# NILOIDE/A.I.gar

Hardware: NVIDIA B200
Metric: env_steps_per_sec (higher is better)
Workload: dtype f64

## Files before the change

a.i.gar_b200/csrc/agar_b200.cu:

```cuda
#include <cuda_runtime.h>
#include <math.h>
#include <stdio.h>
#include <stdlib.h>
#include <string.h>

#include "../../include/agar_b200.h"
#include "../../include/agar_layout.h"
#include "agar_bots.cuh"
#include "agar_dev.cuh"
#include "agar_simple.cuh"

extern __shared__ __align__(16) uint8_t g_smem[];

__device__ __forceinline__ void stage_in(const DevParams& P, const uint8_t* state, int env0, int n_here, bool zero) {
    const int chunks = (int)(P.L.record_bytes / 8);
    const int total = n_here * chunks;
    const uint2* src = (const uint2*)(state + (size_t)env0 * P.L.record_bytes);
    for (int i = threadIdx.x; i < total; i += blockDim.x) {
        int e = i / chunks, w = i - e * chunks;
        uint2 v = zero ? make_uint2(0u, 0u) : src[i];
        ((uint2*)(g_smem + (size_t)e * P.rec_stride))[w] = v;
    }
    __syncthreads();
}
// ... 94 lines not shown
#ifdef AGAR_PHASE_CLOCKS
            c.clk_t = clock64(), c.clk_env = env;
#endif
            if (psync) __syncthreads();
            CLK_MARK(0);
            const int f = n_frames > 0 ? it % n_frames : 0, d = n_frames > 0 ? it / n_frames : 0;
            const bool emit = last || (f == 0 && (flags & KF_OBS_BEFORE));
            if (active && !last && c.lane == 0) c.h->n_events = 0;
            if (FULL && K > 1 && active && !last) {
                update_all_fovs(c, P);
                c.fov_done = true;
                CLK_MARK(8);
                if (K * P.L.cell_cap > W) build_live_cells(c, P);
                CLK_MARK(11);
            }
            for (int k = 0; k < K; ++k) {
                if (psync_bots && k > 0) __syncthreads();
                if (active) {
                    if (!FULL || P.cfg.bot_type[k] == AGAR_BOT_NN) {
                        nn_turn_begin<W, FULL>(c, P, k, (emit && obs_env) ? obs_env + (size_t)k * SL : nullptr);
                        if (last) continue;
                        if (c.lane == 0) {
                            float act[4] = {0.f, 0.f, 0.f, 0.f};
                            if (c.pl[k].bot.need_action) {
                                if (flags & KF_RANDOM_ACTIONS) {
                                    uint32_t w[4];
                                    philox(dec_base + (uint32_t)d, 7u, c.env_id, (uint32_t)k, (uint32_t)P.seed,
                                           (uint32_t)(P.seed >> 32), w);
                                    for (int i = 0; i < 4; ++i) act[i] = (float)(w[i] >> 8) * (1.0f / 16777216.0f);
                                } else {
                                    const float* ap = actions + ((size_t)env * A + k) * 4;
                                    for (int i = 0; i < 4; ++i) act[i] = ap[i];
                                }
                            }
                            nn_turn_end(c, P, k, act);
                        }
                        c.t.sync();
                    } else if (FULL && !last) {
                        CLK_MARK(1);
                        scripted_turn(c, P, k);
                        CLK_MARK(7);
                    }
                }
            }
            if (last) break;
            CLK_MARK(1);
            c.fov_done = false, c.n_live = -1;
            for (int ph = 0; ph < AGAR_FIELD_PHASES; ++ph) {
                if (ph == 0 ? psync : psync_field) __syncthreads();
                if (ph == 0) CLK_MARK(2);
                if (active) field_update_phase<W, FULL>(c, P, ph);
                CLK_MARK(3 + ph);
            }
            if (active) {
                if (c.lane == 0) c.h->frame += 1;
                c.t.sync();
            }
            CLK_MARK(12);
        }
        if (active && c.lane == 0 && (P.turn_reward || P.turn_done))
            for (int a = 0; a < A; ++a) {
                if (P.turn_reward) P.turn_reward[(size_t)env * A + a] = (float)c.pl[a].bot.last_reward;
                if (P.turn_done) P.turn_done[(size_t)env * A + a] = (uint8_t)c.pl[a].bot.exp_done;
            }
    }
    if (P.stage == 1) stage_out(P, state, env0, n_here);
    if (P.stage >= 2) {
        __syncthreads();
        pel_cache_copy(P, state, env0, n_here, tiles, false);
    }
    export_tail(P, obs, env0, n_here);
}


struct SimplePlan {
    int frame_sync;
    int strideB;
    int grid_off;
    int obs_warps;
    int snap_off;
    int snap_stride;
};

enum { SB_PHYS = 1, SB_FULL = 2, SB_EMPTY = 4 };
struct SimpleSnap {
    double fov_x, fov_y, fov_size, mass;
    int32_t out;
    int32_t pad;
};
__host__ __device__ constexpr int simple_max_threads(int W) { return W == 8 ? 352 : 256; }
constexpr int SIMPLE_OBS_MIN_FRAMES = 4;
constexpr int SIMPLE_OBS_LANES = 4;
constexpr int SIMPLE_OBS_WARPS = 4;

template <int ID>
DEV void named_bar_sync(int n) { asm volatile("bar.sync %0, %1;" ::"n"(ID), "r"(n) : "memory"); }
template <int ID>
DEV void named_bar_arrive(int n) { asm volatile("bar.arrive %0, %1;" ::"n"(ID), "r"(n) : "memory"); }

template <int W, bool OBSW>
__global__ void __launch_bounds__(OBSW ? simple_max_threads(W) : 256, W == 1 ? 2 : 1)
k_simple(const __grid_constant__ DevParams P, const SimplePlan SP, uint8_t* __restrict__ state, const float* __restrict__ actions,
         float* __restrict__ obs, int n_frames, int n_dec, int flags, uint32_t dec_base) {
    const int phys_threads = blockDim.x - 32 * SP.obs_warps;
    const int per = phys_threads / W;
    const int env0 = blockIdx.x * per;
    const int n_here = min(per, P.n_envs - env0);
    const int rec_words = (int)(P.L.record_bytes / 4), pel_word = (int)(P.L.off_pellets / 4);
    const int tail_words = rec_words - pel_word;
    {
        for (int i = threadIdx.x; i < per * tail_words; i += blockDim.x) {
            int e = i / tail_words, w = i - e * tail_words;
            int es = e < n_here ? e : n_here - 1;
            const uint32_t* src = (const uint32_t*)(state + (size_t)(env0 + es) * P.L.record_bytes) + pel_word;
            *(uint32_t*)(g_smem + (size_t)e * SP.strideB + w * 4) = src[w];
        }
    }
    __syncthreads();
    auto snap = [&](int buf, int e) { return g_smem + SP.snap_off + (size_t)(buf * per + e) * SP.snap_stride; };
    if (OBSW && (int)threadIdx.x >= phys_threads) {
        constexpr int WO = SIMPLE_OBS_LANES;
        const int ot = ((int)threadIdx.x - phys_threads) / WO, osub = threadIdx.x % WO, n_ot = 32 * SP.obs_warps / WO;
        for (int d = 0; d < n_dec; ++d) {
            const int buf = d & 1;
            if (buf) named_bar_sync<SB_FULL + 1>(blockDim.x);
            else named_bar_sync<SB_FULL>(blockDim.x);
            for (int base = 0; base < per; base += n_ot) {
                const int e = min(base + ot, per - 1);
                const SimpleSnap* sn = (const SimpleSnap*)snap(buf, e);
                SReg r;
                r.fov_x = sn->fov_x, r.fov_y = sn->fov_y, r.fov_size = sn->fov_size, r.mass = sn->mass;
                SPtr q;
                q.pel = (uint32_t*)(sn + 1);
                q.grid = (uint32_t*)(g_smem + (size_t)e * SP.strideB + SP.grid_off);
                const bool out = base + ot < per && sn->out != 0;
                s_encode<WO>(r, q, P, out, out ? obs + (size_t)(env0 + e) * P.L.state_len : nullptr, osub);
            }
            if (d + 2 < n_dec) {
                if (buf) named_bar_arrive<SB_EMPTY + 1>(blockDim.x);
                else named_bar_arrive<SB_EMPTY>(blockDim.x);
            }
        }
        if (flags & KF_OBS_AFTER) __syncthreads();
    } else {
        const int slot = threadIdx.x / W, sub = threadIdx.x % W;
        const bool valid = slot < n_here;
        const int env = env0 + (valid ? slot : n_here - 1);
        const uint32_t env_id = (uint32_t)(P.first_env + (uint64_t)env);
        uint8_t* rec = state + (size_t)env * P.L.record_bytes;
        uint8_t* b = g_smem + (size_t)slot * SP.strideB;
        SPtr q;
        q.h = (AgarEnvHeader*)(rec + P.L.off_header);
        q.p = (AgarPlayer*)(rec + P.L.off_players);
        q.c = (AgarCell*)(rec + P.L.off_cells);
        q.pel = (uint32_t*)b;
        q.ev = (AgarEvent*)(b + (P.L.off_events - P.L.off_pellets));
        q.grid = SP.grid_off ? (uint32_t*)(b + SP.grid_off) : nullptr;
        SReg r;
        s_load(r, q);
        float* row = (obs != nullptr && valid) ? obs + (size_t)env * P.L.state_len : nullptr;
        auto frame_bar = [&]() {
            if (OBSW) named_bar_sync<SB_PHYS>(phys_threads);
            else __syncthreads();
        };
        for (int d = 0; d < n_dec; ++d) {
            if (OBSW && SP.obs_warps) {
                const int d_o = s_turn_begin(r, P);
                if (d_o) s_observe_state(r, P);
                const int buf = d & 1;
                if (d >= 2) {
                    if (buf) named_bar_sync<SB_EMPTY + 1>(blockDim.x);
                    else named_bar_sync<SB_EMPTY>(blockDim.x);
                }
                uint8_t* sn = snap(buf, slot);
                uint32_t* pool = (uint32_t*)(sn + sizeof(SimpleSnap));
                for (int i = sub; i < P.L.pellet_cap; i += W) pool[i] = q.pel[i];
                if (sub == 0) {
                    SimpleSnap* h = (SimpleSnap*)sn;
                    h->fov_x = r.fov_x, h->fov_y = r.fov_y, h->fov_size = r.fov_size, h->mass = r.mass;
                    h->out = d_o != 0 && row != nullptr;
                }
                if (buf) named_bar_arrive<SB_FULL + 1>(blockDim.x);
                else named_bar_arrive<SB_FULL>(blockDim.x);
            } else if (flags & KF_OBS_BEFORE) {
                int d_o = s_turn_begin(r, P);
                s_observe<W>(r, q, P, d_o != 0, row, sub);
            }
            for (int f = 0; f < n_frames; ++f) {
                if (SP.frame_sync == 1 || SP.frame_sync == 4) frame_bar();
                if (SP.frame_sync == 2) __syncwarp();
                r.n_events = 0;
                int d_o = s_turn_begin(r, P);
                s_observe<W>(r, q, P, d_o != 0, nullptr, sub);
                float act[4] = {0.f, 0.f, 0.f, 0.f};
                if (r.need_action) {
                    if (flags & KF_RANDOM_ACTIONS) {
                        uint32_t w[4];
                        philox(dec_base + (uint32_t)d, 7u, env_id, 0u, (uint32_t)P.seed, (uint32_t)(P.seed >> 32), w);
                        for (int i = 0; i < 4; ++i) act[i] = (float)(w[i] >> 8) * (1.0f / 16777216.0f);
                    } else {
                        const float* ap = actions + (size_t)env * 4;
                        for (int i = 0; i < 4; ++i) act[i] = ap[i];
                    }
                }
                double speed_pow;
                s_turn_end<W>(r, P, act, sub, speed_pow);
                if (SP.frame_sync == 4) frame_bar();
                s_field_update<W>(r, q, P, env_id, sub, speed_pow);
            }
        }
        if (flags & KF_OBS_AFTER) {
            if (OBSW) __syncthreads();
            int d_o = s_turn_begin(r, P);
            s_observe<W>(r, q, P, d_o != 0, row, sub);
        }
        if (valid && sub == 0) {
            s_store(r, q);
            if (P.turn_reward) P.turn_reward[env] = (float)r.last_reward;
            if (P.turn_done) P.turn_done[env] = (uint8_t)r.exp_done;
        }
    }
    __syncthreads();
    for (int i = threadIdx.x; i < n_here * tail_words; i += blockDim.x) {
        int e = i / tail_words, w = i - e * tail_words;
        uint32_t* dst = (uint32_t*)(state + (size_t)(env0 + e) * P.L.record_bytes) + pel_word;
        dst[w] = *(const uint32_t*)(g_smem + (size_t)e * SP.strideB + w * 4);
    }
    export_tail(P, obs, env0, n_here);
}

template <int W, bool FULL>
__global__ void __launch_bounds__(1024)
k_init(const __grid_constant__ DevParams P, uint8_t* __restrict__ state, const uint8_t* __restrict__ mask, int mode) {
    const int tiles = blockDim.x / W;
    const int env0 = blockIdx.x * tiles;
    const int n_here = min(tiles, P.n_envs - env0);
    if (P.stage == 1)
        stage_in(P, state, env0, n_here, mode == 0);
    else if (mode == 0) {
        const int chunks = (int)(P.L.record_bytes / 8);
        uint2* dst = (uint2*)(state + (size_t)env0 * P.L.record_bytes);
        for (int i = threadIdx.x; i < n_here * chunks; i += blockDim.x) dst[i] = make_uint2(0u, 0u);
        __syncthreads();
    }
    if (P.stage >= 2) pel_cache_copy(P, state, env0, n_here, tiles, true);
    const int tile_id = threadIdx.x / W;
    if (tile_id < n_here && (mask == nullptr || mode == 0 || mask[env0 + tile_id])) {
        Ctx<W> c(cg::tiled_partition<W>(cg::this_thread_block()));
        bind_ctx(c, P, tile_id, tiles, env0 + tile_id, state);
        const int K = P.L.n_players;
        if (mode == 0 || mode == 1) {
            if (mode == 1) {
                for (int i = c.lane; i < P.L.pellet_cap; i += W) c.pel[i] = 0;
                AgarFatPellet zf = {};
                for (int i = c.lane; i < P.L.fat_cap; i += W) c.fat[i] = zf;
                AgarMote zm = {};
                for (int i = c.lane; i < P.L.blob_cap; i += W) c.blob[i] = zm;
                for (int i = c.lane; i < P.L.virus_cap; i += W) c.vir[i] = zm;
                c.t.sync();
            }
            if (c.lane == 0) {
                if (mode == 0) {
                    for (int k = 0; k < K; ++k) {
                        AgarPlayer* p = &c.pl[k];
                        p->alive = 1;
                        p->cmd_x = p->cmd_y = -1;
                        p->bot.type = P.cfg.bot_type[k];
                    }
                } else {
                    c.h->n_events = 0;
                    c.h->n_pellets = c.h->n_fat = c.h->n_blobs = c.h->n_viruses = 0;
                    c.h->n_dead = 0;
                    for (int i = 0; i < AGAR_MAX_PLAYERS; ++i) c.h->dead_order[i] = 0;
                    for (int k = 0; k < K; ++k)
                        for (int i = 0; i < c.pl[k].n_cells; ++i) CELLP(c, P, k, i)->flags &= ~AGAR_CF_INHASH;
                    c.h->frame = 0;
                }
                c.h->event_hash = 0xCBF29CE484222325ULL;
                for (int k = 0; k < K; ++k) initialize_player(c, P, k);
            }
            c.t.sync();
            spawn_pellets(c, P);
            if (c.lane == 0) {
                if (P.cfg.virus_enabled) spawn_viruses(c, P);
                if (c.h->n_dead) spawn_players(c, P);
            }
            c.t.sync();
        }
        if (mode == 0 || mode == 2) {
            if (c.lane == 0)
                for (int k = 0; k < K; ++k) bot_reset(c, P, k);
            const int nh = P.L.n_agents * P.L.n_hist * P.L.grid_squares * P.L.grid_squares;
// ... 104 lines not shown
    const int max_threads = (e->full && W == 32) ? 1024 : 512;
    int tiles = e->full ? max_threads / W : 128 / W;
    if (getenv("AGAR_MAX_TILES")) tiles = atoi(getenv("AGAR_MAX_TILES"));
    if (tiles * W > max_threads) tiles = max_threads / W;
    while (tiles > 1 && per_tile * tiles > budget) tiles -= 1;
    if (W == 32 && tiles > 4) tiles -= tiles % 4;
    if (per_tile * tiles > budget) return false;
    if (e->full && W == 32 && tiles > 8 && !getenv("AGAR_MAX_TILES")) {
        int sms = 148;
        cudaDeviceGetAttribute(&sms, cudaDevAttrMultiProcessorCount, e->device);
        long long best_cost = -1;
        int best = tiles;
        for (int t = tiles; t >= 8 && t >= tiles - 4; t -= 4) {
            long long ctas = (e->n_envs + t - 1) / t, waves = (ctas + sms - 1) / sms;
            long long cost = waves * t;
            if (best_cost < 0 || cost < best_cost) best_cost = cost, best = t;
        }
        tiles = best;
    }
    e->W = W;
    e->tiles = tiles;
    e->threads = tiles * W;
    e->smem_bytes = per_tile * tiles;
    return true;
}

template <typename K>
static cudaError_t ensure_max_smem(K kernel, int device, unsigned char* done) {
    if (device >= 0 && device < 64 && done[device]) return cudaSuccess;
    int optin = 0;
    cudaError_t err = cudaDeviceGetAttribute(&optin, cudaDevAttrMaxSharedMemoryPerBlockOptin, device);
    if (err != cudaSuccess) return err;
    err = cudaFuncSetAttribute(kernel, cudaFuncAttributeMaxDynamicSharedMemorySize, optin);
    if (err == cudaSuccess && device >= 0 && device < 64) done[device] = 1;
    return err;
}

template <int W, bool FULL, int MAXT>
static cudaError_t launch_main_k(AgarEnv* e, const float* actions, float* obs, int n_frames, int n_dec, int flags,
                                 uint32_t dec_base, cudaStream_t s) {
    static unsigned char done[64];
    cudaError_t err = ensure_max_smem(k_main<W, FULL, MAXT>, e->device, done);
    if (err != cudaSuccess) return err;
    int blocks = (e->n_envs + e->tiles - 1) / e->tiles;
    k_main<W, FULL, MAXT><<<blocks, e->threads, e->smem_bytes, s>>>(e->P, e->state, actions, obs, n_frames, n_dec, flags, dec_base);
    return cudaGetLastError();
}
template <int W, bool FULL>
static cudaError_t launch_main_t(AgarEnv* e, const float* actions, float* obs, int n_frames, int n_dec, int flags,
                                 uint32_t dec_base, cudaStream_t s) {
    if (W == 32 && FULL && e->threads > 768) return launch_main_k<32, true, 1024>(e, actions, obs, n_frames, n_dec, flags, dec_base, s);
    if (W == 32 && FULL && e->threads > 512) return launch_main_k<32, true, 768>(e, actions, obs, n_frames, n_dec, flags, dec_base, s);
    return launch_main_k<W, FULL, 512>(e, actions, obs, n_frames, n_dec, flags, dec_base, s);
}
template <int W, bool FULL>
static cudaError_t launch_init_t(AgarEnv* e, const uint8_t* mask, int mode, cudaStream_t s) {
    static unsigned char done[64];
    cudaError_t err = ensure_max_smem(k_init<W, FULL>, e->device, done);
    if (err != cudaSuccess) return err;
    int blocks = (e->n_envs + e->init_tiles - 1) / e->init_tiles;
    k_init<W, FULL><<<blocks, e->init_threads, e->init_smem, s>>>(e->P, e->state, mask, mode);
    return cudaGetLastError();
}
#define DISPATCH(fn, ...)                                                 \
    (e->full ? (e->W == 32  ? fn<32, true>(__VA_ARGS__)                   \
                : e->W == 16 ? fn<16, true>(__VA_ARGS__)                  \
                : e->W == 8  ? fn<8, true>(__VA_ARGS__)                   \
                             : fn<4, true>(__VA_ARGS__))                  \
             : (e->W == 32  ? fn<32, false>(__VA_ARGS__)                  \
                             : fn<32, false>(__VA_ARGS__)))

static int launch_main(AgarEnv* e, const float* actions, float* obs, int n_frames, int n_dec, int flags, uint32_t dec_base,
                       void* stream) {
    AgarEnv* env = e;
    CU(cudaSetDevice(e->device));
    cudaError_t err;
    if (e->simple_W) {
        const bool handoff = e->obs_threads && (flags & KF_OBS_BEFORE) && obs != nullptr && n_frames >= SIMPLE_OBS_MIN_FRAMES;
        const SimplePlan& sp = handoff ? e->sp_obs : e->sp;
        const int threads = handoff ? e->obs_threads : e->simple_threads;
        const size_t smem = handoff ? e->obs_smem : e->simple_smem;
        const int per = (threads - 32 * sp.obs_warps) / e->simple_W;
        if (threads % 32 || threads > (handoff ? simple_max_threads(e->simple_W) : 256) || per < 1 || per * e->simple_W % 32 ||
            (sp.obs_warps && (!sp.grid_off || 32 * sp.obs_warps % SIMPLE_OBS_LANES)))
            return fail(e, AGAR_E_INVALID, "inconsistent k_simple launch shape%s", "");
        int blocks = (e->n_envs + per - 1) / per;
#define LAUNCH_SIMPLE(WW, OB)                                                                                                 \
    do {                                                                                                                      \
        static unsigned char done_##WW##OB[64];                                                                               \
        err = ensure_max_smem(k_simple<WW, OB>, e->device, done_##WW##OB);                                                    \
        if (err == cudaSuccess) {                                                                                             \
            k_simple<WW, OB><<<blocks, threads, smem, (cudaStream_t)stream>>>(e->P, sp, e->state, actions, obs, n_frames,     \
                                                                              n_dec, flags, dec_base);                        \
            err = cudaGetLastError();                                                                                         \
        }                                                                                                                     \
    } while (0)
        if (handoff && e->simple_W == 4) LAUNCH_SIMPLE(4, true);
        else if (handoff) LAUNCH_SIMPLE(8, true);
        else if (e->simple_W == 1) LAUNCH_SIMPLE(1, false);
        else if (e->simple_W == 2) LAUNCH_SIMPLE(2, false);
        else if (e->simple_W == 4) LAUNCH_SIMPLE(4, false);
        else if (e->simple_W == 8) LAUNCH_SIMPLE(8, false);
        else if (e->simple_W == 16) LAUNCH_SIMPLE(16, false);
        else LAUNCH_SIMPLE(32, false);
#undef LAUNCH_SIMPLE
        if (handoff && err == cudaSuccess) e->observer_launches += 1;
    } else
        err = DISPATCH(launch_main_t, e, actions, obs, n_frames, n_dec, flags, dec_base, (cudaStream_t)stream);
    if (err != cudaSuccess) return fail(e, AGAR_E_CUDA, "kernel launch failed: %s", cudaGetErrorString(err));
    e->launches += 1;
    return AGAR_OK;
}
static int launch_init(AgarEnv* e, const uint8_t* mask, int mode, void* stream) {
    AgarEnv* env = e;
    CU(cudaSetDevice(e->device));
    cudaError_t err = e->full ? (e->init_W == 32 ? launch_init_t<32, true>(e, mask, mode, (cudaStream_t)stream)
                                                  : launch_init_t<8, true>(e, mask, mode, (cudaStream_t)stream))
                              : launch_init_t<32, false>(e, mask, mode, (cudaStream_t)stream);
    if (err != cudaSuccess) return fail(e, AGAR_E_CUDA, "kernel launch failed: %s", cudaGetErrorString(err));
    e->launches += 1;
    return AGAR_OK;
}

template <int W, bool OBSW>
static int simple_ctas_per_sm(int device, int threads, size_t smem) {
    static unsigned char done[64];
    int n = 0;
    if (ensure_max_smem(k_simple<W, OBSW>, device, done) != cudaSuccess ||
        cudaOccupancyMaxActiveBlocksPerMultiprocessor(&n, k_simple<W, OBSW>, threads, smem) != cudaSuccess) {
        cudaGetLastError();
        return 0;
    }
    return n;
}

static void plan_observers(AgarEnv* e) {
    e->obs_threads = 0;
    e->sp_obs = e->sp;
    const int W = e->simple_W;
    if ((W != 4 && W != 8) || !e->sp.grid_off || e->L.pellet_cap > 64 * SIMPLE_OBS_LANES) return;
    if (cudaSetDevice(e->device) != cudaSuccess) {
        cudaGetLastError();
        return;
    }
    int sms = 148;
    cudaDeviceGetAttribute(&sms, cudaDevAttrMultiProcessorCount, e->device);
    const int per_warp = 32 / W;
    const int K = SIMPLE_OBS_WARPS;
    int warps = ((e->n_envs + sms - 1) / sms + per_warp - 1) / per_warp;
    if (warps > simple_max_threads(W) / 32 - K) warps = simple_max_threads(W) / 32 - K;
    const int per = warps * per_warp;
    const size_t env_bytes = ((size_t)per * e->sp.strideB + 15) / 16 * 16;
    const int snap_stride = (int)((sizeof(SimpleSnap) + (size_t)e->L.pellet_cap * 4 + 15) / 16 * 16);
    const size_t smem = env_bytes + 2 * (size_t)per * snap_stride;
    if (smem > 200 * 1024) return;
    const int threads = (warps + K) * 32;
    const int occ = W == 8 ? simple_ctas_per_sm<8, true>(e->device, threads, smem) : simple_ctas_per_sm<4, true>(e->device, threads, smem);
    const int occ_in = W == 8 ? simple_ctas_per_sm<8, false>(e->device, e->simple_threads, e->simple_smem)
                              : simple_ctas_per_sm<4, false>(e->device, e->simple_threads, e->simple_smem);
    if (occ < 1 || occ_in < 1) return;
    const long long per_in = e->simple_threads / W;
    const long long waves = ((e->n_envs + per - 1) / per + (long long)sms * occ - 1) / ((long long)sms * occ);
    const long long waves_in = ((e->n_envs + per_in - 1) / per_in + (long long)sms * occ_in - 1) / ((long long)sms * occ_in);
    if (waves > waves_in) return;
    e->sp_obs.obs_warps = K;
    e->sp_obs.snap_off = (int)env_bytes;
    e->sp_obs.snap_stride = snap_stride;
    e->obs_threads = threads;
    e->obs_smem = smem;
}

extern "C" int agar_set_tile_width(AgarEnv* e, int W) {
    if (!e) return AGAR_E_INVALID;
    if (!e->full && e->L.grid_squares <= 16 && (W == 1 || W == 2 || W == 4 || W == 8 || W == 16 || W == 32) &&
        !getenv("AGAR_GENERAL_KERNEL")) {
        int tail_words = (int)((e->L.record_bytes - e->L.off_pellets) / 4);
        e->sp.strideB = (tail_words | 1) * 4;
        e->sp.grid_off = 0;
        e->sp.obs_warps = e->sp.snap_off = e->sp.snap_stride = 0;
        const char* genv = getenv("AGAR_SIMPLE_OBS_SMEM");
        if (genv ? atoi(genv) != 0 : W >= 2) {
            const int gg = e->L.grid_squares * e->L.grid_squares;
            e->sp.grid_off = tail_words * 4;
            e->sp.strideB = ((tail_words + gg) | 1) * 4;
        }
        if (e->L.pellet_cap > (W >= 4 ? 64 : 128) * W)
            return fail(e, AGAR_E_UNSUPPORTED, "pellet pool too large for this tile width%s", "");
        int threads = 128;
        const char* tenv = getenv("AGAR_SIMPLE_THREADS");
        if (tenv && atoi(tenv) >= 32) threads = atoi(tenv) / 32 * 32;
        if (threads > 256) threads = 256;
        e->sp.frame_sync = getenv("AGAR_SIMPLE_SYNC") ? atoi(getenv("AGAR_SIMPLE_SYNC")) : 1;
        size_t per_env = (size_t)e->sp.strideB;
        while (threads > 32 && per_env * (threads / W) > 200 * 1024) threads -= 32;
        if (per_env * (threads / W) > 200 * 1024)
            return fail(e, AGAR_E_NOMEM, "pellet pool + event ring of %s do not fit in shared memory at this tile width", "the envs of one CTA");
        e->simple_W = W;
        e->simple_threads = threads;
        e->simple_smem = per_env * (threads / W);
        e->W = W;
        plan_observers(e);
        return AGAR_OK;
    }
    bool ok = W == 32 || (e->full && (W == 4 || W == 8 || W == 16));
    if (!ok) return fail(e, AGAR_E_INVALID, "unsupported tile width%s", "");
    if (!plan_launch(e, W)) return fail(e, AGAR_E_NOMEM, "env record does not fit in shared memory%s", "");
    e->simple_W = 0;
    return AGAR_OK;
}
extern "C" int agar_get_tile_width(const AgarEnv* e) { return e ? e->W : 0; }

extern "C" int agar_create(const AgarConfig* cfg, int n_envs, int device, uint64_t seed, uint64_t first_env_id, void* stream,
                           AgarEnv** out) {
    AgarEnv* env = nullptr;
    if (!cfg || !out || n_envs < 1) return fail(nullptr, AGAR_E_INVALID, "bad arguments to agar_create%s", "");
    AgarLayout L;
    int rc = agar_layout_compute(cfg, &L);
    if (rc != AGAR_OK) return fail(nullptr, rc, "config rejected by agar_layout_compute%s", "");
    int ndev = 0;
    if (cudaGetDeviceCount(&ndev) != cudaSuccess || device < 0 || device >= ndev)
        return fail(nullptr, AGAR_E_CUDA, "no such CUDA device%s", "");
    CU(cudaSetDevice(device));
    AgarEnv* e = (AgarEnv*)calloc(1, sizeof(AgarEnv));
    env = e;
    e->cfg = *cfg;
    e->L = L;
    e->n_envs = n_envs;
    e->device = device;
    e->full = config_is_simple(*cfg, L) ? 0 : 1;
    DevParams& P = e->P;
    memset(&P, 0, sizeof P);
    P.cfg = *cfg;
    P.L = L;
    P.S = L.field_size;
    P.nb = (int)ceil((double)P.S / AG_BUCKET);
    P.n_envs = n_envs;
    P.rec_stride = (int)L.record_bytes + 8;
// ... 255 lines not shown
```

a.i.gar_b200/csrc/agar_simple.cuh:

```cuda
#pragma once
#include "agar_bots.cuh"
#include "agar_dev.cuh"

#define S_FULL 0xffffffffu
#define S_NONE 0x7fffffff

struct SReg {
    uint32_t rng_field, frame;
    int32_t n_pellets, n_events;
    uint64_t event_hash;
    double cmd_x, cmd_y, fov_x, fov_y, fov_size;
    int32_t fov_valid;
    double x, y, mass, radius, svx, svy, merge_time;
    int32_t counter;
    uint32_t uid, flags;
    int32_t has_action, has_last_action, skip_frames, has_last_mass, has_old_state, time, skipping, turn_begun, need_action,
        exp_valid, exp_done;
    double a0, a1, a2, a3, l0, l1, l2, l3;
    double cum_reward, last_reward, last_mass, fov_size_feat, stat_mass_sum, stat_mass_max, stat_frames;
};

struct SPtr {
    AgarEnvHeader* h;
    AgarPlayer* p;
// ... 73 lines not shown
    philox(r.rng_field, 0u, env_id, 0, (uint32_t)P.seed, (uint32_t)(P.seed >> 32), w);
    r.rng_field += 1;
    return lo + (int)(((unsigned long long)w[0] * (unsigned long long)(hi - lo)) >> 32);
}
DEV void s_update_fov(SReg& r, const DevParams& P) {
    double tm = 0.0 + r.mass;
    if (tm != 0) {
        r.fov_x = (0.0 + r.x * r.mass) / tm;
        r.fov_y = (0.0 + r.y * r.mass) / tm;
        r.fov_valid = 1;
    }
    r.fov_size = agar_pow(r.radius, 0.475) * P.pow_n[1] * 35;
}
template <int W>
DEV void s_dual_pow(double x0, double y0, double x1, double y1, int sub, double& p0, double& p1) {
    if (W == 1) {
        p0 = agar_pow(x0, y0);
        p1 = agar_pow(x1, y1);
        return;
    }
    const bool odd = (sub & 1) != 0;
    const double mine = agar_pow(odd ? x1 : x0, odd ? y1 : y0);
    const double other = __shfl_xor_sync(S_FULL, mine, 1);
    p0 = odd ? other : mine;
    p1 = odd ? mine : other;
}
template <int W>
DEV void s_dual_div(double a, double b, double c, double d, int sub, double& q0, double& q1) {
    if (W == 1) {
        q0 = a / b;
        q1 = c / d;
        return;
    }
    const bool odd = (sub & 1) != 0;
    const double mine = (odd ? c : a) / (odd ? d : b);
    const double other = __shfl_xor_sync(S_FULL, mine, 1);
    q0 = odd ? other : mine;
    q1 = odd ? mine : other;
}
template <int W>
DEV void s_set_command_point(SReg& r, const DevParams& P, double a0, double a1, int sub, double& speed_pow) {
    double tm = 0.0 + r.mass;
    {
        double fx, fy;
        s_dual_div<W>(0.0 + r.x * r.mass, tm, 0.0 + r.y * r.mass, tm, sub, fx, fy);
        if (tm != 0) {
            r.fov_x = fx;
            r.fov_y = fy;
            r.fov_valid = 1;
        }
    }
    const double mass_next = r.mass >= 4 ? r.mass * P.decay_rate : r.mass;
    double fov_pow;
    s_dual_pow<W>(r.radius, 0.475, mass_next, -0.35, sub, fov_pow, speed_pow);
    r.fov_size = fov_pow * P.pow_n[1] * 35;
    int x = (int)r.fov_x, y = (int)r.fov_y;
    int left = x - (int)(r.fov_size / 2), top = y - (int)(r.fov_size / 2);
    int size = (int)r.fov_size;
    r.cmd_x = left + a0 * size;
    r.cmd_y = top + a1 * size;
}

template <int W>
struct SMask {
    typedef uint32_t T;
    static constexpr int MB = 32;
};
template <>
struct SMask<1> {
    typedef unsigned long long T;
    static constexpr int MB = 64;
};
template <>
struct SMask<2> {
    typedef unsigned long long T;
    static constexpr int MB = 64;
};
DEV int s_ffs(uint32_t m) { return __ffs((int)m); }
DEV int s_ffs(unsigned long long m) { return __ffsll((long long)m); }

DEV void s_observe_state(SReg& r, const DevParams& P) {
    s_update_fov(r, P);
    r.fov_size_feat = P.cfg.use_fovsize ? r.fov_size : r.fov_size_feat;
}

template <int W>
DEV void s_encode(const SReg& r, const SPtr& q, const DevParams& P, bool out, float* row, int sub) {
    const int G = P.L.grid_squares, GG = G * G, SL = P.L.state_len;
    const double S = (double)P.S;
    if (!s_any<W>(out)) return;
    const bool staged = q.grid != nullptr;
    if (out) {
        if (staged)
            for (int i = sub; i < GG; i += W) q.grid[i] = 0u;
        else
            for (int i = sub; i < GG; i += W) row[i] = 0.f;
        if (sub == 0) {
            int n = GG;
            if (P.cfg.use_fovsize) row[n++] = (float)r.fov_size;
            if (P.cfg.use_totalmass) row[n++] = (float)(0.0 + r.mass);
            (void)SL;
        }
    }
    s_sync<W>();
    if (out) {
        const double fov = r.fov_size, fx = r.fov_x, fy = r.fov_y;
        const double left = fx - fov / 2, top = fy - fov / 2;
        const double gs = fov / G, inv = 1.0 / gs;
        const bool canon = P.cfg.obs_mode == AGAR_OBS_CANONICAL;
        const int cols = canon ? G : (int)ceil(fov / gs);
        double mx = left + gs / 2, my = top + gs / 2;
        unsigned col_bad = 0, row_bad = 0;
        for (int i = 0; i < G; ++i) {
            if (mx + gs / 2 < 0 || mx - gs / 2 > S) col_bad |= 1u << i;
            if (my + gs / 2 < 0 || my - gs / 2 > S) row_bad |= 1u << i;
            mx += gs;
            my += gs;
        }
        const Rect ra = rect_of(P.S, fx, fy, fov / 2);
        const double h = fov / 2;
        const double xmin = fx - h, xmax = fx + h, ymin = fy - h, ymax = fy + h;
        const int wx0 = (int)floor(xmin) - 1, wx1 = (int)ceil(xmax) + 1, wy0 = (int)floor(ymin) - 1, wy1 = (int)ceil(ymax) + 1;
        typedef typename SMask<W>::T MT;
        constexpr int MB = SMask<W>::MB;
        MT m0 = 0, m1 = 0;
        {
            const int cap = P.L.pellet_cap, split = min(cap, sub + MB * W);
            int j = 0;
            for (int s = sub; s < split; s += W, ++j) {
                uint32_t pk = q.pel[s];
                int px = AGAR_PELLET_X(pk), py = AGAR_PELLET_Y(pk);
                bool in = px >= wx0 && px <= wx1 && py >= wy0 && py <= wy1 && pk != 0;
                m0 |= (MT)in << j;
            }
            j = 0;
            for (int s = sub + MB * W; s < cap; s += W, ++j) {
                uint32_t pk = q.pel[s];
                int px = AGAR_PELLET_X(pk), py = AGAR_PELLET_Y(pk);
                bool in = px >= wx0 && px <= wx1 && py >= wy0 && py <= wy1 && pk != 0;
                m1 |= (MT)in << j;
            }
        }
        const bool sheared = cols != G;
        const bool use_bits = W <= 2 && !canon && G <= 15;
        const unsigned edges = use_bits ? edge_bits(gs, inv, G) : 0u;
        while (m0 | m1) {
            int j;
            if (m0) {
                j = s_ffs(m0) - 1;
                m0 &= m0 - 1;
            } else {
                j = MB + s_ffs(m1) - 1;
                m1 &= m1 - 1;
            }
            uint32_t pk = q.pel[sub + W * j];
            int px = AGAR_PELLET_X(pk), py = AGAR_PELLET_Y(pk), pm = AGAR_PELLET_M(pk);
            double pr = P.pellet_r[pm & 3];
            double dx = (double)px, dy = (double)py;
            bool ok = rect_hit(ra, pellet_rect(px, py)) && !(dx + pr < xmin || dx - pr > xmax || dy + pr < ymin || dy - pr > ymax);
            int c0, c1, r0, r1;
            if (use_bits) {
                axis_buckets2_bits(dx - left, pr, fov, gs, inv, edges, c0, c1);
                axis_buckets2_bits(dy - top, pr, fov, gs, inv, edges, r0, r1);
            } else {
                axis_buckets2(dx - left, pr, fov, gs, inv, canon, c0, c1);
                axis_buckets2(dy - top, pr, fov, gs, inv, canon, r0, r1);
// ... 208 lines not shown
```

Before: 1.124 billion.

## Restructure observer warps into window/cull/compacted-bin/scatter phases across all lanes

Replaces the per-env 4-lane s_encode in the dedicated observer warps with a multi-phase pipeline. Each thread first computes a per-env view window. Warps then cull pellets with ballots and prefix sums into a shared compacted candidate list, all observer threads bin candidates into the grid with shared atomics, and the result is scattered to obs. This aims to balance work across observer threads and skip pellets outside the window, at the cost of extra named barriers, atomics and more shared memory per block, which may lower occupancy. It also adds optional clock64 phase instrumentation, compiled out by default.

```diff
diff --git a/a.i.gar_b200/csrc/agar_b200.cu b/a.i.gar_b200/csrc/agar_b200.cu
--- a/a.i.gar_b200/csrc/agar_b200.cu
+++ b/a.i.gar_b200/csrc/agar_b200.cu
@@ -200,7 +200,7 @@
     int snap_stride;
 };
 
-enum { SB_PHYS = 1, SB_FULL = 2, SB_EMPTY = 4 };
+enum { SB_PHYS = 1, SB_FULL = 2, SB_EMPTY = 4, SB_OBS = 6 };
 struct SimpleSnap {
     double fov_x, fov_y, fov_size, mass;
     int32_t out;
@@ -208,8 +208,19 @@
 };
 __host__ __device__ constexpr int simple_max_threads(int W) { return W == 8 ? 352 : 256; }
 constexpr int SIMPLE_OBS_MIN_FRAMES = 4;
-constexpr int SIMPLE_OBS_LANES = 4;
 constexpr int SIMPLE_OBS_WARPS = 4;
+
+#ifdef AGAR_PHASE_CLOCKS
+enum { SCLK_PHYS_EMPTY, SCLK_PHYS_FRAMES, SCLK_OBS_FULL, SCLK_OBS_PASS, SCLK_N_EMPTY, SCLK_N_FRAMES, SCLK_N_PASSES };
+#define SCLK(t) const long long t = clock64()
+#define SCLK_ADD(slot, v)                                                                                     \
+    do {                                                                                                      \
+        if ((threadIdx.x & 31) == 0) atomicAdd(&g_clk[(size_t)blockIdx.x * 16 + (slot)], (unsigned long long)(v)); \
+    } while (0)
+#else
+#define SCLK(t) do { } while (0)
+#define SCLK_ADD(slot, v) do { } while (0)
+#endif
 
 template <int ID>
 DEV void named_bar_sync(int n) { asm volatile("bar.sync %0, %1;" ::"n"(ID), "r"(n) : "memory"); }
@@ -237,27 +248,84 @@
     __syncthreads();
     auto snap = [&](int buf, int e) { return g_smem + SP.snap_off + (size_t)(buf * per + e) * SP.snap_stride; };
     if (OBSW && (int)threadIdx.x >= phys_threads) {
-        constexpr int WO = SIMPLE_OBS_LANES;
-        const int ot = ((int)threadIdx.x - phys_threads) / WO, osub = threadIdx.x % WO, n_ot = 32 * SP.obs_warps / WO;
+        const int n_ot = 32 * SP.obs_warps, ot = (int)threadIdx.x - phys_threads, lane = ot & 31;
+        const int G = P.L.grid_squares, GG = G * G, cap = P.L.pellet_cap;
+        const bool canon = P.cfg.obs_mode == AGAR_OBS_CANONICAL;
+        const bool use_bits = !canon && G <= 15;
+        SObsWin* win = (SObsWin*)snap(2, 0);
+        unsigned* n_cand = (unsigned*)(win + per);
+        unsigned* cand = n_cand + 1;
+        auto grid = [&](int e) { return (uint32_t*)(g_smem + (size_t)e * SP.strideB + SP.grid_off); };
+        auto pool = [&](int buf, int e) { return (const uint32_t*)(snap(buf, e) + sizeof(SimpleSnap)); };
+        auto obs_bar = [&]() { named_bar_sync<SB_OBS>(n_ot); };
         for (int d = 0; d < n_dec; ++d) {
             const int buf = d & 1;
+            SCLK(t0);
             if (buf) named_bar_sync<SB_FULL + 1>(blockDim.x);
             else named_bar_sync<SB_FULL>(blockDim.x);
-            for (int base = 0; base < per; base += n_ot) {
-                const int e = min(base + ot, per - 1);
+            SCLK(t1);
+            for (int e = ot; e < per; e += n_ot) {
                 const SimpleSnap* sn = (const SimpleSnap*)snap(buf, e);
-                SReg r;
-                r.fov_x = sn->fov_x, r.fov_y = sn->fov_y, r.fov_size = sn->fov_size, r.mass = sn->mass;
-                SPtr q;
-                q.pel = (uint32_t*)(sn + 1);
-                q.grid = (uint32_t*)(g_smem + (size_t)e * SP.strideB + SP.grid_off);
-                const bool out = base + ot < per && sn->out != 0;
-                s_encode<WO>(r, q, P, out, out ? obs + (size_t)(env0 + e) * P.L.state_len : nullptr, osub);
+                if (!sn->out) continue;
+                win[e] = s_obs_window(P, sn->fov_x, sn->fov_y, sn->fov_size);
+                float* row = obs + (size_t)(env0 + e) * P.L.state_len + GG;
+                if (P.cfg.use_fovsize) *row++ = (float)sn->fov_size;
+                if (P.cfg.use_totalmass) *row = (float)(0.0 + sn->mass);
+            }
+            if (ot == 0) *n_cand = 0;
+            obs_bar();
+            for (int e = ot >> 5; e < per; e += SP.obs_warps) {
+                if (!((const SimpleSnap*)snap(buf, e))->out) continue;
+                SObsWin& w = win[e];
+                if (use_bits) {
+                    bool f0 = false, f1 = false;
+                    if (lane <= G) {
+                        const double x0 = (double)lane * w.gs, x1 = x0 + w.gs;
+                        f0 = bucket_of_edge(x0, w.gs, w.inv) != lane;
+                        f1 = bucket_of_edge(x1, w.gs, w.inv) != lane + 1;
+                    }
+                    const unsigned b0 = __ballot_sync(S_FULL, f0), b1 = __ballot_sync(S_FULL, f1);
+                    if (lane == 0) w.edges = b0 | b1 << 16;
+                }
+                uint32_t* g = grid(e);
+                for (int i = lane; i < GG; i += 32) g[i] = 0u;
+                const uint32_t* pl = pool(buf, e);
+                unsigned m = 0;
+                for (int s = lane, j = 0; s < cap; s += 32, ++j) m |= (unsigned)s_in_window(w, pl[s]) << j;
+                const int c = __popc(m);
+                int incl = c;
+#pragma unroll
+                for (int off = 1; off < 32; off <<= 1) {
+                    const int v = __shfl_up_sync(S_FULL, incl, off);
+                    if (lane >= off) incl += v;
+                }
+                unsigned base = 0;
+                if (lane == 31) base = atomicAdd(n_cand, (unsigned)incl);
+                base = __shfl_sync(S_FULL, base, 31) + (unsigned)(incl - c);
+                for (; m; m &= m - 1) cand[base++] = (unsigned)e << 16 | (unsigned)(lane + 32 * (__ffs((int)m) - 1));
+            }
+            obs_bar();
+            const int n = (int)*n_cand;
+            for (int i = ot; i < n; i += n_ot) {
+                const unsigned ce = cand[i];
+                const int e = (int)(ce >> 16);
+                uint32_t* g = grid(e);
+                s_bin_pellet(win[e], pool(buf, e)[ce & 0xffff], P, use_bits, canon,
+                             [&](int id, int pm) { atomicAdd(&g[id], (unsigned)pm); });
+            }
+            obs_bar();
+            for (int e = ot / GG, k = ot % GG; e < per;) {
+                if (((const SimpleSnap*)snap(buf, e))->out) obs[(size_t)(env0 + e) * P.L.state_len + k] = (float)grid(e)[k];
+                for (k += n_ot; k >= GG; k -= GG) ++e;
             }
             if (d + 2 < n_dec) {
                 if (buf) named_bar_arrive<SB_EMPTY + 1>(blockDim.x);
                 else named_bar_arrive<SB_EMPTY>(blockDim.x);
             }
+            SCLK(t2);
+            SCLK_ADD(SCLK_OBS_FULL, t1 - t0);
+            SCLK_ADD(SCLK_OBS_PASS, t2 - t1);
+            SCLK_ADD(SCLK_N_PASSES, 1);
         }
         if (flags & KF_OBS_AFTER) __syncthreads();
     } else {
@@ -287,8 +355,12 @@
                 if (d_o) s_observe_state(r, P);
                 const int buf = d & 1;
                 if (d >= 2) {
+                    SCLK(t0);
                     if (buf) named_bar_sync<SB_EMPTY + 1>(blockDim.x);
                     else named_bar_sync<SB_EMPTY>(blockDim.x);
+                    SCLK(t1);
+                    SCLK_ADD(SCLK_PHYS_EMPTY, t1 - t0);
+                    SCLK_ADD(SCLK_N_EMPTY, 1);
                 }
                 uint8_t* sn = snap(buf, slot);
                 uint32_t* pool = (uint32_t*)(sn + sizeof(SimpleSnap));
@@ -304,6 +376,7 @@
                 int d_o = s_turn_begin(r, P);
                 s_observe<W>(r, q, P, d_o != 0, row, sub);
             }
+            SCLK(tf0);
             for (int f = 0; f < n_frames; ++f) {
                 if (SP.frame_sync == 1 || SP.frame_sync == 4) frame_bar();
                 if (SP.frame_sync == 2) __syncwarp();
@@ -326,6 +399,9 @@
                 if (SP.frame_sync == 4) frame_bar();
                 s_field_update<W>(r, q, P, env_id, sub, speed_pow);
             }
+            SCLK(tf1);
+            SCLK_ADD(SCLK_PHYS_FRAMES, tf1 - tf0);
+            SCLK_ADD(SCLK_N_FRAMES, n_frames);
         }
         if (flags & KF_OBS_AFTER) {
             if (OBSW) __syncthreads();
@@ -596,7 +672,7 @@
         const size_t smem = handoff ? e->obs_smem : e->simple_smem;
         const int per = (threads - 32 * sp.obs_warps) / e->simple_W;
         if (threads % 32 || threads > (handoff ? simple_max_threads(e->simple_W) : 256) || per < 1 || per * e->simple_W % 32 ||
-            (sp.obs_warps && (!sp.grid_off || 32 * sp.obs_warps % SIMPLE_OBS_LANES)))
+            (sp.obs_warps && !sp.grid_off))
             return fail(e, AGAR_E_INVALID, "inconsistent k_simple launch shape%s", "");
         int blocks = (e->n_envs + per - 1) / per;
 #define LAUNCH_SIMPLE(WW, OB)                                                                                                 \
@@ -652,7 +728,7 @@
     e->obs_threads = 0;
     e->sp_obs = e->sp;
     const int W = e->simple_W;
-    if ((W != 4 && W != 8) || !e->sp.grid_off || e->L.pellet_cap > 64 * SIMPLE_OBS_LANES) return;
+    if ((W != 4 && W != 8) || !e->sp.grid_off) return;
     if (cudaSetDevice(e->device) != cudaSuccess) {
         cudaGetLastError();
         return;
@@ -666,7 +742,7 @@
     const int per = warps * per_warp;
     const size_t env_bytes = ((size_t)per * e->sp.strideB + 15) / 16 * 16;
     const int snap_stride = (int)((sizeof(SimpleSnap) + (size_t)e->L.pellet_cap * 4 + 15) / 16 * 16);
-    const size_t smem = env_bytes + 2 * (size_t)per * snap_stride;
+    const size_t smem = env_bytes + 2 * (size_t)per * snap_stride + (size_t)per * sizeof(SObsWin) + 4 * (1 + (size_t)per * e->L.pellet_cap);
     if (smem > 200 * 1024) return;
     const int threads = (warps + K) * 32;
     const int occ = W == 8 ? simple_ctas_per_sm<8, true>(e->device, threads, smem) : simple_ctas_per_sm<4, true>(e->device, threads, smem);
diff --git a/a.i.gar_b200/csrc/agar_simple.cuh b/a.i.gar_b200/csrc/agar_simple.cuh
--- a/a.i.gar_b200/csrc/agar_simple.cuh
+++ b/a.i.gar_b200/csrc/agar_simple.cuh
@@ -179,6 +179,68 @@
 DEV void s_observe_state(SReg& r, const DevParams& P) {
     s_update_fov(r, P);
     r.fov_size_feat = P.cfg.use_fovsize ? r.fov_size : r.fov_size_feat;
+}
+
+struct SObsWin {
+    double left, top, fov, gs, inv, xmax, ymax;
+    Rect ra;
+    int wx0, wx1, wy0, wy1;
+    unsigned col_bad, row_bad;
+    unsigned edges;
+    int sheared;
+};
+DEV SObsWin s_obs_window(const DevParams& P, double fx, double fy, double fov) {
+    const int G = P.L.grid_squares;
+    const double S = (double)P.S;
+    SObsWin w;
+    w.fov = fov;
+    w.left = fx - fov / 2, w.top = fy - fov / 2;
+    w.gs = fov / G, w.inv = 1.0 / w.gs;
+    const int cols = P.cfg.obs_mode == AGAR_OBS_CANONICAL ? G : (int)ceil(fov / w.gs);
+    w.sheared = cols != G;
+    double mx = w.left + w.gs / 2, my = w.top + w.gs / 2;
+    w.col_bad = w.row_bad = 0;
+    for (int i = 0; i < G; ++i) {
+        if (mx + w.gs / 2 < 0 || mx - w.gs / 2 > S) w.col_bad |= 1u << i;
+        if (my + w.gs / 2 < 0 || my - w.gs / 2 > S) w.row_bad |= 1u << i;
+        mx += w.gs;
+        my += w.gs;
+    }
+    w.ra = rect_of(P.S, fx, fy, fov / 2);
+    const double h = fov / 2;
+    w.xmax = fx + h, w.ymax = fy + h;
+    w.wx0 = (int)floor(w.left) - 1, w.wx1 = (int)ceil(w.xmax) + 1, w.wy0 = (int)floor(w.top) - 1, w.wy1 = (int)ceil(w.ymax) + 1;
+    w.edges = 0;
+    return w;
+}
+DEV bool s_in_window(const SObsWin& w, uint32_t pk) {
+    const int px = AGAR_PELLET_X(pk), py = AGAR_PELLET_Y(pk);
+    return px >= w.wx0 && px <= w.wx1 && py >= w.wy0 && py <= w.wy1 && pk != 0;
+}
+template <class Put>
+DEV void s_bin_pellet(const SObsWin& w, uint32_t pk, const DevParams& P, bool use_bits, bool canon, Put put) {
+    const int G = P.L.grid_squares;
+    int px = AGAR_PELLET_X(pk), py = AGAR_PELLET_Y(pk), pm = AGAR_PELLET_M(pk);
+    double pr = P.pellet_r[pm & 3];
+    double dx = (double)px, dy = (double)py;
+    bool ok = rect_hit(w.ra, pellet_rect(px, py)) && !(dx + pr < w.left || dx - pr > w.xmax || dy + pr < w.top || dy - pr > w.ymax);
+    int c0, c1, r0, r1;
+    if (use_bits) {
+        axis_buckets2_bits(dx - w.left, pr, w.fov, w.gs, w.inv, w.edges, c0, c1);
+        axis_buckets2_bits(dy - w.top, pr, w.fov, w.gs, w.inv, w.edges, r0, r1);
+    } else {
+        axis_buckets2(dx - w.left, pr, w.fov, w.gs, w.inv, canon, c0, c1);
+        axis_buckets2(dy - w.top, pr, w.fov, w.gs, w.inv, canon, r0, r1);
+    }
+    auto cell = [&](int cc, int rr) {
+        int sr = w.sheared ? cc + rr : cc, sc = rr;
+        if (sr >= G) sr -= G, sc += 1;
+        if (ok && cc >= 0 && rr >= 0 && sc < G && !((w.row_bad >> sc & 1) || (w.col_bad >> sr & 1))) put(sr + sc * G, pm);
+    };
+    cell(c0, r0);
+    cell(c1, r0);
+    cell(c0, r1);
+    cell(c1, r1);
 }
 
 template <int W>
```

After: 1.149 billion (median of 6 runs). +2.3%, better.
